# ziatdinovmax/pyroVED

Measured on AMD Instinct MI355X. Metric: images/sec (SVI step), higher is better.
Workload: dtype bf16; 1 GPU; C2 iVAE 28x28 invariances=['r','t'] latent_dim=2 bernoulli, batch 256 per GPU (global 256), bf16 MFMA operands for the hidden-layer contractions (fp32 accumulate; fp32 elsewhere); the guide (fc encoder, sample, split) runs in the decoder launch's prologue in fp32, SVI step = ELBO+grads+Adam; parallelism=dp1

## Files before the change

pyroved_amd/csrc/pv_sdec_fused_w8.hip:

```cpp
#include "pv_sdec_fused.h"
#include "pv_fb_layout.h"
#include "pv_sdec_prims.h"
#include "pv_kernels.h"
#include <stdlib.h>

#define W8_WAVES 8
#define W8_ROWS (W8_WAVES * FD_UNIT)
#define W8_THREADS (64 * W8_WAVES)
#define W8_ARR (W8_ROWS * LDS2)
#define W8_ARR_BYTES (2 * W8_ARR)
#define WO_W1 0
#define WO_W2 IMG_BYTES
#define WO_SA (2 * IMG_BYTES)
#define WO_SB (WO_SA + W8_ARR_BYTES)
#define WO_VEC (WO_SB + W8_ARR_BYTES)
#define WO_ATAB (WO_VEC + 3 * FD_H * 4)
#define WO_TTAB (WO_ATAB + 8 * 64 * 8)
#define WO_INFO (WO_TTAB + 4 * 64 * 16)
#define WO_RED (WO_INFO + 3 * W8_ROWS * 4)
#define WO_CHZ (WO_RED + 256)
#define WO_CTP (WO_CHZ + W8_WAVES * FD_H * 4)
#define WO_CGR (WO_CTP + W8_WAVES * 256)
#define W8_LDS_BYTES (WO_CGR + W8_WAVES * 256)
#define WO_TX (WO_SB + 2 * 32 * LDS2)
// ... 2 lines not shown
static_assert(WO_TLOG + W8_WAVES * 16 * 4 <= WO_SB + W8_ARR_BYTES, "tail exchange buffers fit behind the staged rows");
static_assert(W8_LDS_BYTES <= 160 * 1024, "LDS budget");
static_assert(2 * IMG_BYTES % (W8_WAVES * 1024) == 0, "image load: whole 1 KB LDS-DMA pieces per wave");

#ifndef W8_FENCE_MASK
#define W8_FENCE_MASK 0
#endif
#define W8_FENCE() __builtin_amdgcn_sched_barrier(W8_FENCE_MASK)

__device__ __forceinline__ float w8_tanhc(float cx) {
  const float e = __builtin_amdgcn_exp2f(cx);
  return 1.0f - 2.0f * __builtin_amdgcn_rcpf(e + 1.0f);
}
#ifndef W8_HSWAP
#define W8_HSWAP 0
#endif
#ifndef W8_QSWAP
#define W8_QSWAP 1
#endif
bool pv_sdec_fused_w8_qswap() { return W8_QSWAP != 0; }
__device__ __forceinline__ bf16x8 w8_catq(const bf16x4& a, const bf16x4& b, int q) {
  return W8_QSWAP ? sd_catq(a, b, q >= 2) : sd_cat(a, b);
}
__device__ __forceinline__ float w8_sum_q(float v) {
  return pv_sum_rows(v);
}

#ifndef W8_ABL
#define W8_ABL 0
#endif
#ifndef W8_TAIL
#define W8_TAIL 1
#endif
#define W8_ABL_LOADS(bit, g) (!(W8_ABL & (bit)) || (((g) & 1) == 0))
#define W8_ABL_BUF(bit, g) ((W8_ABL & (bit)) ? (((g) >> 1) & 1) : ((g) & 1))


struct W8Addr : SdAddr { int fs, hs; };
__device__ __forceinline__ W8Addr w8_addr(int r, int q) {
  W8Addr a;
  a.fs = W8_HSWAP ? ((r >> 2) & 1) : 0;
  a.hs = W8_HSWAP ? (q & 1) : (W8_QSWAP ? ((r >> 1) & 1) : 0);
  static_cast<SdAddr&>(a) = sd_addr(r, q);
  return a;
}

__device__ __forceinline__ void w8_layer_fwd(const __bf16* __restrict__ Wh, const float* __restrict__ bs,
                                             const bf16x4 (&ih)[8], f32x4 (&out)[8], const W8Addr& ad, int q) {
#pragma unroll
  for (int ob = 0; ob < 8; ++ob) out[ob] = *reinterpret_cast<const f32x4*>(bs + 16 * ob + 4 * q);
  const __bf16* ah = Wh + ad.fb;
#if W8_HSWAP
  const __bf16* ah0 = ah + 4 * ad.fs;
  const __bf16* ah1 = ah + 4 - 4 * ad.fs;
  asm volatile("" : "+v"(ah0), "+v"(ah1));
#endif
  const int (&xm)[4] = ad.fx;
  bf16x8 wh[2][2];
  auto load = [&](int g, bf16x8 (&h)[2]) {
    const int m = g >> 2, op = (g & 3) * 2;
#pragma unroll
    for (int o = 0; o < 2; ++o) {
#if W8_HSWAP
      typedef const volatile bf16x4* vp4;
      const bf16x4 lo4 = *reinterpret_cast<vp4>(ah0 + 16 * (op + o) * LDB + xm[m]);
      const bf16x4 hi4 = *reinterpret_cast<vp4>(ah1 + 16 * (op + o) * LDB + xm[m]);
// ... 183 lines not shown
}
__device__ __forceinline__ f32x4 w8_tanh4(f32x4 v) {
#pragma unroll
  for (int i = 0; i < 4; ++i) v[i] = w8_tanhc(v[i]);
  return v;
}
__device__ __forceinline__ bf16x4 w8_cvt4(const f32x4& v) {
  bf16x4 h;
#pragma unroll
  for (int i = 0; i < 4; ++i) h[i] = (__bf16)v[i];
  return h;
}
__device__ __forceinline__ f32x4 w8_mul_dtanh4(const f32x4& d, const bf16x4& hb) {
  const f32x4 t = sd_f32_of(hb);
  return d * (t * t - 1.0f);
}

#define WF_H1 WO_SA
#define WF_H2 (WF_H1 + 512)
#define WF_HD (WF_H2 + 512)
#define WF_P (WF_HD + 512)
#define WF_P_WAVE (64 * 17 * 4)
static_assert(WF_P + W8_WAVES * WF_P_WAVE <= WO_VEC, "guide scratch fits in the staging arrays");
#include "pv_gemv16.h"

#define W8_COOP_SPINS 4096
__device__ unsigned w8_coop_late_total;
extern "C" int pv_debug_coop_late_count(unsigned* out) {
  return (int)hipMemcpyFromSymbol(out, HIP_SYMBOL(w8_coop_late_total), sizeof(unsigned));
}
template <bool GRADS, int LIK, int FOLDK>
__global__ __launch_bounds__(W8_THREADS) void pv_sdec_w8_kernel(PvFused f, PvEncFold e) {
  constexpr bool FOLD = FOLDK != 0, CHAIN = FOLDK >= 2, COOP = FOLDK == 3;
  extern __shared__ __attribute__((aligned(16))) char smb[];
  const int tid = threadIdx.x, lane0 = tid & 63, lane = lane0, r = lane & 15, q = lane >> 4;
  const int wave = __builtin_amdgcn_readfirstlane(tid >> 6);
  const int g = blockIdx.x, G = gridDim.x;
  const unsigned lds0 = __builtin_amdgcn_readfirstlane((unsigned)(size_t)smb);
  const __bf16* W1h = reinterpret_cast<const __bf16*>(smb + WO_W1);
  const __bf16* W2h = reinterpret_cast<const __bf16*>(smb + WO_W2);
  __bf16* sA = reinterpret_cast<__bf16*>(smb + WO_SA);
  __bf16* sB = reinterpret_cast<__bf16*>(smb + WO_SB);
  float* vec = reinterpret_cast<float*>(smb + WO_VEC);
  float* info = reinterpret_cast<float*>(smb + WO_INFO);
  float* red = reinterpret_cast<float*>(smb + WO_RED);
  const char* gimg = reinterpret_cast<const char*>(f.wimg);
  W8_STAMP_K(0);
  f32x4 xr[4], xpk;
  f32x4 xc[4][4];
  unsigned coop_tag = 0;
  if (COOP) {
    coop_tag = e.coop_flags[G] + 1u;
    const int K4 = (int)(e.ldx >> 2);
#pragma unroll
    for (int i = 0; i < 4; ++i) {
      const float* xg = e.x + (int64_t)(8 * (4 * wave + i) + (g & 7)) * e.ldx;
#pragma unroll
      for (int c = 0; c < 4; ++c) {
        const int k4 = lane + 64 * c;
        xc[i][c] = *reinterpret_cast<const f32x4*>(xg + 4 * (k4 < K4 ? k4 : 0));
      }
    }
  }
  if (FOLD && !COOP) {
    const int K4 = (int)(e.ldx >> 2);
    const float* xg = e.x + (int64_t)g * e.ldx;
#pragma unroll
    for (int c = 0; c < 4; ++c) {
      const int k4 = lane + 64 * c;
      xr[c] = *reinterpret_cast<const f32x4*>(xg + 4 * (k4 < K4 ? k4 : 0));
    }
    const int kp = 64 * (((K4 + 63) >> 6) - 1) + (lane & 3);
    xpk = *reinterpret_cast<const f32x4*>(xg + 4 * (kp < K4 ? kp : 0));
  }
  float pt_v[3] = {0.0f, 0.0f, 0.0f}, pt_a = 0.0f, pt_t[8] = {0.0f, 0.0f, 0.0f, 0.0f, 0.0f, 0.0f, 0.0f, 0.0f};
  if (FOLD) {
    if (tid < FD_H) { pt_v[0] = f.wo[tid]; pt_v[1] = f.b1[tid]; pt_v[2] = f.b2[tid]; }
    {
      const int jb = tid >> 6, m = lane & 15, kq = lane >> 4, j = 16 * jb + m;
      if (kq == 0) pt_a = f.Wc[j * f.cd];
      else if (kq == 1) pt_a = f.cd == 2 ? f.Wc[j * 2 + 1] : 0.0f;
      else if (kq == 2) pt_a = f.bc[j];
    }
    if (tid < 256) {
      const int mm = tid >> 6, m = lane & 15, kq = lane >> 4;
#pragma unroll
      for (int e_ = 0; e_ < 8; ++e_) {
        const int j = 32 * mm + 4 * kq + (e_ < 4 ? e_ : 16 + e_ - 4);
        if (m < 2) pt_t[e_] = f.Wc[j * f.cd];
        else if (m < 4 && f.cd == 2) pt_t[e_] = f.Wc[j * 2 + 1];
      }
    }
  }

  f32x4 w1v[8], w2v[8];
  if (!FOLD) {
    constexpr int PIECES = IMG_BYTES / (W8_WAVES * 1024);
#pragma unroll
    for (int c = 0; c < PIECES; ++c) {
      const int off = (wave * PIECES + c) * 1024;
      sd_glds16(gimg + off + lane * 16, lds0 + WO_W1 + off);
      sd_glds16(gimg + 2 * IMG_BYTES + off + lane * 16, lds0 + WO_W2 + off);
    }
  } else {
    if (GRADS) {
      const int64_t b0 = (int64_t)g * e.img_per_wg;
      f32x4* zp = reinterpret_cast<f32x4*>(f.part_hz + b0 * f.kmax * FD_H);
      const int n4 = e.img_per_wg * f.kmax * (FD_H / 4);
      for (int i = tid; i < n4; i += W8_THREADS) zp[i] = f32x4{0.0f, 0.0f, 0.0f, 0.0f};
      if (f.part_rs) {
        f32x4* zr = reinterpret_cast<f32x4*>(f.part_rs + b0 * f.kmax * PV_RS_W);
        for (int i = tid; i < e.img_per_wg * f.kmax * (PV_RS_W / 4); i += W8_THREADS) zr[i] = f32x4{0.0f, 0.0f, 0.0f, 0.0f};
      }
    }
  }
  if (FOLD) {
    float* h1s = reinterpret_cast<float*>(smb + WF_H1);
    float* h2s = reinterpret_cast<float*>(smb + WF_H2);
    float* hds = reinterpret_cast<float*>(smb + WF_HD);
    float* zs = hds + 64;
    float* P = reinterpret_cast<float*>(smb + WF_P + wave * WF_P_WAVE);
    const int N = (int)e.ldx, zd = e.z_dim;
    const int r_ = lane & 15, q_ = lane >> 4;
    {
      const int64_t b = g;
      const int jw = 16 * wave + r_;
      const float pb1 = (e.enc1.b_off >= 0 && jw < e.enc1.out_dim) ? e.params[e.enc1.b_off + jw] : 0.0f;
      const float pbh = (e.head.b_off >= 0 && jw < e.head.out_dim) ? e.params[e.head.b_off + jw] : 0.0f;
      const float pep = (wave == 0 && lane < zd) ? e.eps[b * zd + lane] : 0.0f;
      f32x4 wl1[8], wlh[8];
      float pwz[4] = {0.0f, 0.0f, 0.0f, 0.0f};
      if (tid < FD_H) {
#pragma unroll
        for (int i = 0; i < 4; ++i) pwz[i] = i < e.lat_in ? e.Wz[(int64_t)tid * e.lat_in + i] : 0.0f;
      }
      auto layer0_alone = [&](const f32x4 (&xr_)[4], const f32x4& xpk_, bool load_next) {
        const int jr = 16 * ((wave + g) & (W8_WAVES - 1));
        const float v = w8_gemv16(e.params + e.enc0.w_off, N, e.enc0.out_dim, jr, xr_, xpk_, P, lane,
// ... 155 lines not shown
      }
      pv_lds_barrier();
      if (tid < FD_H) {
        int coord = 0;
        if (e.coord_dim == 1) coord = e.has_t ? 1 : 0;
        else if (e.coord_dim == 2) coord = e.has_r + 2 * e.has_t + e.has_s;
        const float* wz = e.Wz + (int64_t)tid * e.lat_in;
        float v = 0.0f;
        for (int i = 0; i < e.lat_in; ++i) v += zs[coord + i] * (i < 4 ? pwz[i] : wz[i]);
        e.hz[b * FD_H + tid] = v * SD_C;
      }
      W8_STAMP_K(7);
    }
  }
  if (tid < FD_H) {
    vec[tid] = FOLD ? pt_v[0] : f.wo[tid];
    vec[FD_H + tid] = SD_C * (FOLD ? pt_v[1] : f.b1[tid]);
    vec[2 * FD_H + tid] = SD_C * (FOLD ? pt_v[2] : f.b2[tid]);
  }
  {
    const int jb = tid >> 6, m = lane & 15, kq = lane >> 4, j = 16 * jb + m;
    float v = 0.0f;
    if (FOLD) v = SD_C * pt_a;
    else if (kq == 0) v = SD_C * f.Wc[j * f.cd];
    else if (kq == 1) v = f.cd == 2 ? SD_C * f.Wc[j * 2 + 1] : 0.0f;
    else if (kq == 2) v = SD_C * f.bc[j];
    __bf16 hi, lo;
    fb_split(v, hi, lo);
    bf16x4 a = sd_zero4();
    if (kq < 2) { a[0] = hi; a[1] = hi; a[2] = lo; }
    else if (kq == 2) { a[0] = hi; a[1] = lo; }
    reinterpret_cast<bf16x4*>(smb + WO_ATAB)[tid] = a;
  }
  if (tid < 256) {
    const int mm = tid >> 6, m = lane & 15, kq = lane >> 4;
    bf16x8 a;
#pragma unroll
    for (int e = 0; e < 8; ++e) {
      const int j = 32 * mm + 4 * kq + (e < 4 ? e : 16 + e - 4);
      float w = 0.0f;
      if (FOLD) w = pt_t[e];
      else if (m < 2) w = f.Wc[j * f.cd];
      else if (m < 4 && f.cd == 2) w = f.Wc[j * 2 + 1];
      __bf16 hi, lo;
      fb_split(w, hi, lo);
      a[e] = m >= 4 ? (__bf16)0.0f : ((m & 1) ? lo : hi);
    }
    reinterpret_cast<bf16x8*>(smb + WO_TTAB)[tid] = a;
  }
  if (FOLD) {
    typedef unsigned short us4 __attribute__((ext_vector_type(4)));
    __bf16* i1 = reinterpret_cast<__bf16*>(smb + WO_W1);
    __bf16* i2 = reinterpret_cast<__bf16*>(smb + WO_W2);
#pragma unroll
    for (int u = 0; u < 8; ++u) {
      const int idx = tid + W8_THREADS * u, row = idx >> 5, c4 = idx & 31;
      us4 h1, h2;
#pragma unroll
      for (int i = 0; i < 4; ++i) {
        h1[i] = __builtin_bit_cast(unsigned short, (__bf16)(w1v[u][i] * SD_C));
        h2[i] = __builtin_bit_cast(unsigned short, (__bf16)(w2v[u][i] * SD_C));
      }
      const int el = fb_wel(row, fb_pcol(4 * c4)) ^ (W8_HSWAP ? 4 * ((row >> 2) & 1) : 0) ^ (W8_QSWAP ? 4 * ((c4 >> 1) & 1) : 0);
      *reinterpret_cast<us4*>(i1 + el) = h1;
      *reinterpret_cast<us4*>(i2 + el) = h2;
    }
  }
  sd_wait_vm0();
  __syncthreads();
  W8_STAMP_K(1);
  const float bo = f.bo[0];
  typedef __attribute__((address_space(1))) float gfloat;
  unsigned long long u_llrow, u_loc, u_rowtp, u_part_hz;
  int64_t a_M;
  asm volatile("s_mov_b64 %0, %5\n\ts_mov_b64 %1, %6\n\ts_mov_b64 %2, %7\n\ts_mov_b64 %3, %8\n\ts_mov_b64 %4, %9"
               : "=&s"(u_llrow), "=&s"(u_loc), "=&s"(u_rowtp), "=&s"(u_part_hz), "=&s"(a_M)
               : "s"((unsigned long long)f.llrow), "s"((unsigned long long)f.loc), "s"((unsigned long long)f.rowtp),
                 "s"((unsigned long long)f.part_hz), "s"(f.M));
  gfloat* a_llrow = (gfloat*)u_llrow; gfloat* a_loc = (gfloat*)u_loc; gfloat* a_rowtp = (gfloat*)u_rowtp;
  gfloat* a_part_hz = (gfloat*)u_part_hz;

  f32x4 accW1[2][4], accW2[2][4], accS[8], accB1 = {0, 0, 0, 0}, accB2 = {0, 0, 0, 0};
#pragma unroll
  for (int kb = 0; kb < 8; ++kb) {
    accW1[kb >> 2][kb & 3] = f32x4{0, 0, 0, 0}; accW2[kb >> 2][kb & 3] = f32x4{0, 0, 0, 0}; accS[kb] = f32x4{0, 0, 0, 0};
  }
  float dbo = 0.0f;
  int cur_b = -1;
  const int upb = f.N / FD_UNIT;
  float* rec = f.part + (int64_t)g * FD_REC;

  auto flush_hz = [&](int b) {
    const int64_t ub = (int64_t)b * upb;
    const int gfirst = (int)(((ub + 1) * G + f.units - 1) / f.units) - 1;
    gfloat* dst = a_part_hz + ((int64_t)b * f.kmax + (g - gfirst) * W8_WAVES + wave) * FD_H + 4 * q;
    if (r == 0) {
#pragma unroll
      for (int jb = 0; jb < 8; ++jb) *(__attribute__((address_space(1))) f32x4*)(dst + 16 * jb) = accS[jb] * SD_RC2;
    }
#pragma unroll
    for (int jb = 0; jb < 8; ++jb)
#pragma unroll
      for (int i = 0; i < 4; ++i) accS[jb][i] = r == 0 ? 0.0f : accS[jb][i];
  };

  const int u_lo = (int)((int64_t)g * f.units / G), u_hi = (int)((int64_t)(g + 1) * f.units / G);
  const int xun = (int)f.x_units;
  struct Pos { int unit, b, loc, xu; };
  auto pos_of = [&](int unit_) {
    Pos p_;
    p_.unit = unit_; p_.b = unit_ / upb; p_.loc = unit_ - p_.b * upb; p_.xu = xun > 0 ? unit_ % xun : unit_;
    return p_;
  };
  auto advance = [&](Pos& p_, int by) {
    p_.unit += by; p_.loc += by; p_.xu += by;
    while (p_.loc >= upb) { p_.loc -= upb; ++p_.b; }
    if (xun > 0) { while (p_.xu >= xun) p_.xu -= xun; }
  };
  const bool has_tail = W8_TAIL && ((u_hi - u_lo) & (W8_WAVES - 1)) == 1;
  const int u_end = has_tail ? u_hi - 1 : u_hi;
  const Pos pos_lo = pos_of(has_tail ? u_end : u_lo);
  Pos pos_cur = pos_of(u_lo + wave < u_end ? u_lo + wave : (has_tail ? u_end : u_lo));
  Pos pos_nx = pos_cur;
  float sw_next = 1.0f;
  auto x_of = [&](const Pos& p_) -> float {
    if (f.sw) sw_next = f.sw[p_.b];
    return f.x[(int64_t)p_.xu * FD_UNIT + r];
  };
  float xv_next = x_of(pos_cur);
  float* chz = reinterpret_cast<float*>(smb + WO_CHZ) + wave * FD_H;
  float* ctp = reinterpret_cast<float*>(smb + WO_CTP) + wave * 64;
  float* cgr = reinterpret_cast<float*>(smb + WO_CGR) + wave * 64;
  auto fetch_unit_inputs = [&](const Pos& p_) {
    const int n0 = p_.loc * FD_UNIT;
    sd_glds4(f.hz + (int64_t)p_.b * FD_H + lane, lds0 + WO_CHZ + wave * (FD_H * 4));
    sd_glds4(f.hz + (int64_t)p_.b * FD_H + 64 + lane, lds0 + WO_CHZ + wave * (FD_H * 4) + 256);
    sd_glds4(f.tp + (int64_t)p_.b * 8 + (lane & 7), lds0 + WO_CTP + wave * 256);
    sd_glds4(f.grid + (int64_t)n0 * f.cd + (lane & (16 * f.cd - 1)), lds0 + WO_CGR + wave * 256);
  };
  fetch_unit_inputs(pos_cur);
  const W8Addr wad = w8_addr(r, q);
  int tile_no = -1;
  for (int ut = u_lo; ut < u_end; ut += W8_WAVES) {
    ++tile_no;
    (void)tile_no;
    asm volatile("; W8_TILE_BEGIN");
    W8_STAMP(0);
    const int nact = (u_end - ut) < W8_WAVES ? (u_end - ut) : W8_WAVES;
    if (ut + W8_WAVES + wave < u_end) advance(pos_nx, W8_WAVES);
    else pos_nx = pos_lo;
    int opq = 0;
    asm volatile("" : "+v"(opq));
    const int lane = lane0 | opq, r = lane & 15, q = lane >> 4;
    const float* wos = vec;
    const float* b1s = vec + FD_H;
    const float* b2s = vec + 2 * FD_H;
    const bool act = wave < nact;
    const int unit = act ? pos_cur.unit : ut;
    const int bu = pos_cur.b;
    const int64_t row = (int64_t)unit * FD_UNIT + r;
    float x0, x1, u0c, u1c, sc;
    sd_wait_vm0();
    {
      const float* t = ctp;
      const float* gr = cgr;
      if (f.cd == 2) {
        const float gx = gr[2 * r], gy = gr[2 * r + 1];
        u0c = gx * t[0] - gy * t[1];
        u1c = gx * t[1] + gy * t[0];
        sc = t[2];
        x0 = u0c * sc + t[3];
        x1 = u1c * sc + t[4];
      } else {
// ... 12 lines not shown
    {
      bf16x4 bx = sd_zero4();
      {
        const float v = q == 0 ? x0 : x1;
        __bf16 vh, vl;
        fb_split(v, vh, vl);
        const __bf16 one = (__bf16)1.0f;
        if (q < 2) { bx[0] = vh; bx[1] = vl; bx[2] = vh; }
        else if (q == 2) { bx[0] = one; bx[1] = one; }
      }
      const bf16x4* atab = reinterpret_cast<const bf16x4*>(smb + WO_ATAB) + lane;
      const float* hzb = chz;
      bf16x4 aop[8];
#pragma unroll
      for (int jb = 0; jb < 8; ++jb) {
        tC[jb] = *reinterpret_cast<const f32x4*>(hzb + 16 * jb + 4 * q);
        aop[jb] = atab[64 * jb];
      }
      if (GRADS && q == 0) { inf_x0[r] = x0; inf_x1[r] = x1; }
      W8_FENCE();
      if (f.hz_scale == 0.0f) {
#pragma unroll
        for (int jb = 0; jb < 8; ++jb) tC[jb] = tC[jb] * SD_C;
      }
      W8_FENCE();
#pragma unroll
      for (int jb = 0; jb < 8; ++jb) tC[jb] = sd_mfma16(aop[jb], bx, tC[jb]);
      W8_FENCE();
      sd_tanh8<W8_FENCE_MASK>(tC);
      w8_cvt8(tC, h0b);
    }
    asm volatile("; W8_P1_coord_done");
    W8_STAMP(1);
    fetch_unit_inputs(pos_nx);
    {
      w8_layer_fwd(W1h, b1s, h0b, tC, wad, q);
      sd_tanh8<W8_FENCE_MASK>(tC);
      w8_cvt8(tC, h1b);
      asm volatile("; W8_P2_l1_done");
    W8_STAMP(2);
      w8_layer_fwd(W2h, b2s, h1b, tC, wad, q);
      sd_tanh8<W8_FENCE_MASK>(tC);
      f32x4 part4 = {0.0f, 0.0f, 0.0f, 0.0f};
#pragma unroll
      for (int jb = 0; jb < 8; ++jb) {
        const f32x4 wv = *reinterpret_cast<const f32x4*>(wos + 16 * jb + 4 * q);
        part4 = part4 + tC[jb] * wv;
        if (GRADS) {
#pragma unroll
          for (int i = 0; i < 4; ++i) pA[jb][i] = (__bf16)tC[jb][i];
          const f32x4 t2 = tC[jb] * tC[jb];
          tC[jb] = wv - wv * t2;
        }
      }
      const float a = w8_sum_q((part4[0] + part4[1]) + (part4[2] + part4[3])) + bo;
      float ll, locv;
      sd_pixel_lik<LIK>(a, xv, f.sig, f.sigmoid_out, ll, dlda, locv);
      dlda *= act ? swv : 0.0f;
      if (q == 0) {
        if (act) {
          if (a_llrow) a_llrow[row] = ll;
          if (a_loc) a_loc[row] = locv;
        }
        if (GRADS) { dbo += dlda; inf_dl[r] = dlda; }
      }
      xv_next = x_of(pos_nx);
    }
    pos_cur = pos_nx;
    asm volatile("; W8_P3_fwd_done");
    W8_STAMP(3);
    if (!GRADS) continue;
    const int ksteps = (nact + 1) >> 1;
    {
      sd_wait_lgkm0();
      const f32x4 d4 = *reinterpret_cast<const f32x4*>(inf_dl + 4 * q);
      bf16x4 bw = sd_zero4();
#pragma unroll
      for (int i = 0; i < 4; ++i) {
        __bf16 hi, lo;
        fb_split(d4[i], hi, lo);
        bw[i] = r == 3 ? hi : (r == 4 ? lo : (__bf16)0.0f);
      }
      w8_colsum_mfma(sA, pA, bw, accS, wave, r, q);
#pragma unroll
      for (int jb = 0; jb < 8; ++jb) tC[jb] = tC[jb] * dlda;
      w8_cvt8(tC, pA);
    }
    asm volatile("; W8_P4_dwo_done");
    W8_STAMP(4);
    sd_stage_store(sA, pA, 16 * wave + r, q);
    sd_stage_store(sB, h1b, 16 * wave + r, q);
    __syncthreads();
    asm volatile("; W8_P5_bar1");
    W8_STAMP(5);
    w8_wgrad_consume(sA, sB, accW2, accB2, wave, r, q, ksteps);
    asm volatile("; W8_P6_cons2");
    W8_STAMP(6);
    bf16x4 p0[8];
    {
      w8_layer_dgrad(W2h, pA, tC, wad);
      w8_mul_dtanh(tC, h1b);
      w8_cvt8(tC, pA);
      asm volatile("; W8_P7_dgrad2");
    W8_STAMP(7);
      w8_layer_dgrad(W1h, pA, tC, wad);
      w8_mul_dtanh(tC, h0b);
      w8_cvt8(tC, p0);
    }
    asm volatile("; W8_P8_dgrad1");
    W8_STAMP(8);
    __syncthreads();
    W8_STAMP(9);
    {
      f32x4 dd = {0.0f, 0.0f, 0.0f, 0.0f};
      const bf16x8* ttab = reinterpret_cast<const bf16x8*>(smb + WO_TTAB) + lane;
#pragma unroll
      for (int mm = 0; mm < 4; ++mm) dd = MFMA32(ttab[64 * mm], sd_cat(p0[2 * mm], p0[2 * mm + 1]), dd);
      if (q == 0 && act) {
        const float d0 = (dd[0] + dd[1]) * SD_RC2, d1 = (dd[2] + dd[3]) * SD_RC2;
        a_rowtp[row] = sc * (d1 * u0c - d0 * u1c);
        a_rowtp[a_M + row] = d0 * u0c + d1 * u1c;
        a_rowtp[2 * a_M + row] = d0;
        a_rowtp[3 * a_M + row] = d1;
      }
      if (act && bu != cur_b) {
        if (cur_b >= 0) flush_hz(cur_b);
        cur_b = bu;
      }
      const f32x4 a0 = *reinterpret_cast<const f32x4*>(inf_x0 + 4 * q);
      const f32x4 a1 = *reinterpret_cast<const f32x4*>(inf_x1 + 4 * q);
      bf16x4 bc_ = sd_zero4();
      const bool use1 = r == 2 || r == 6, lo_col = r >= 5;
#pragma unroll
      for (int i = 0; i < 4; ++i) {
        __bf16 hi, lo;
        fb_split(use1 ? a1[i] : a0[i], hi, lo);
        __bf16 v = lo_col ? lo : hi;
        if (r == 0) v = (__bf16)1.0f;
        if (r == 3 || r == 4 || r > 6) v = (__bf16)0.0f;
        bc_[i] = v;
      }
      w8_colsum_mfma(sA, p0, bc_, accS, wave, r, q);
      sd_wait_lgkm0();
    }
    asm volatile("; W8_P12_rowlocal");
    W8_STAMP(12);
    sd_stage_store(sA, pA, 16 * wave + r, q);
    sd_stage_store(sB, h0b, 16 * wave + r, q);
    __syncthreads();
    asm volatile("; W8_P10_bar3");
    W8_STAMP(10);
    w8_wgrad_consume(sA, sB, accW1, accB1, wave, r, q, ksteps);
    asm volatile("; W8_P11_cons1");
    W8_STAMP(11);
    __syncthreads();
    asm volatile("; W8_P13_bar4");
    W8_STAMP(13);
    W8_STAMP(14);
    asm volatile("; W8_TILE_END");
  }
// ... 65 lines not shown
      }
      float* tlog = reinterpret_cast<float*>(smb + WO_TLOG);
      if (q == 0) tlog[16 * wave + r] = part;
      __syncthreads();
      float a = bo;
      {
        float sacc = 0.0f;
#pragma unroll
        for (int w = 0; w < W8_WAVES; ++w) sacc += tlog[16 * w + r];
        a += sacc;
      }
      float ll, locv;
      if (LIK == PV_LIK_BERNOULLI) {
        const float pr = sd_rcp(1.0f + sd_exp(-a));
        const float pc = fminf(fmaxf(pr, BERN_EPS), 1.0f - BERN_EPS);
        const float lpc = sd_log(pc), l1pc = sd_log(1.0f - pc);
        const float lg = lpc - l1pc;
        ll = -(fmaxf(lg, 0.0f) - lg * xv - fmaxf(lpc, l1pc));
        const float mask = (pr >= BERN_EPS && pr <= 1.0f - BERN_EPS) ? 1.0f : 0.0f;
        dlda = (pc - xv) * mask;
        locv = pr;
      } else if (LIK == PV_LIK_CBERNOULLI) {
        pv_cbern(a, xv, ll, dlda, locv);
      } else {
        const float pr = f.sigmoid_out ? sd_rcp(1.0f + sd_exp(-a)) : a;
        const float d = xv - pr;
        ll = -(d * d) / (2.0f * f.sig * f.sig) - sd_log(f.sig) - LOG_SQRT_2PI;
        dlda = -d / (f.sig * f.sig) * (f.sigmoid_out ? pr * (1.0f - pr) : 1.0f);
        locv = pr;
      }
      dlda *= swv;
      if (q == 0) {
        if (wave == 0) {
          if (a_llrow) a_llrow[row] = ll;
          if (a_loc) a_loc[row] = locv;
          if (GRADS) dbo += dlda;
        }
        if (GRADS) inf_dl[r] = dlda;
      }
    }
    if (GRADS) {
      bf16x4 pA[8];
      w8_xchg_put(smb, 3, w8_cvt4(gq * dlda), wave, lane);
      __syncthreads();
      w8_xchg_get(smb, 3, pA, lane);
      if (wave == 0) {
        sd_stage_store(sA, pA, r, q);
        sd_stage_store(sB, h1b, r, q);
      } else if (wave == 1) {
        bf16x4 z8[8];
#pragma unroll
        for (int jb = 0; jb < 8; ++jb) z8[jb] = sd_zero4();
        sd_stage_store(sA, z8, 16 + r, q);
        sd_stage_store(sB, h1b, 16 + r, q);
      } else if (wave == 3) {
        bf16x4 h2b[8];
        w8_xchg_get(smb, 2, h2b, lane);
        sd_wait_lgkm0();
        const f32x4 d4 = *reinterpret_cast<const f32x4*>(inf_dl + 4 * q);
        bf16x4 bw = sd_zero4();
#pragma unroll
        for (int i = 0; i < 4; ++i) {
          __bf16 hi, lo;
          fb_split(d4[i], hi, lo);
          bw[i] = r == 3 ? hi : (r == 4 ? lo : (__bf16)0.0f);
        }
        w8_colsum_mfma(sA, h2b, bw, accS, wave, r, q);
      }
      const f32x4 d1 = w8_mul_dtanh4(w8_tail_dgrad(W2h, pA, wad, wave, r), own1);
      w8_xchg_put(smb, 4, w8_cvt4(d1), wave, lane);
      __syncthreads();
      w8_xchg_get(smb, 4, pA, lane);
      w8_wgrad_consume(sA, sB, accW2, accB2, wave, r, q, 1);
      const f32x4 d0 = w8_mul_dtanh4(w8_tail_dgrad(W1h, pA, wad, wave, r), own0);
      w8_xchg_put(smb, 5, w8_cvt4(d0), wave, lane);
      __syncthreads();
      if (wave == 0) {
        sd_stage_store(sA, pA, r, q);
        sd_stage_store(sB, h0b, r, q);
      } else if (wave == 1) {
        bf16x4 z8[8];
#pragma unroll
        for (int jb = 0; jb < 8; ++jb) z8[jb] = sd_zero4();
        sd_stage_store(sA, z8, 16 + r, q);
        sd_stage_store(sB, h0b, 16 + r, q);
      } else if (wave == 2) {
        bf16x4 p0[8];
        w8_xchg_get(smb, 5, p0, lane);
        f32x4 dd = {0.0f, 0.0f, 0.0f, 0.0f};
        const bf16x8* ttab = reinterpret_cast<const bf16x8*>(smb + WO_TTAB) + lane;
#pragma unroll
        for (int mm = 0; mm < 4; ++mm) dd = MFMA32(ttab[64 * mm], sd_cat(p0[2 * mm], p0[2 * mm + 1]), dd);
        if (q == 0) {
          const float d0_ = (dd[0] + dd[1]) * SD_RC2, d1_ = (dd[2] + dd[3]) * SD_RC2;
          a_rowtp[row] = sc * (d1_ * u0c - d0_ * u1c);
          a_rowtp[a_M + row] = d0_ * u0c + d1_ * u1c;
          a_rowtp[2 * a_M + row] = d0_;
          a_rowtp[3 * a_M + row] = d1_;
        }
      } else if (wave == 3) {
        bf16x4 p0[8];
        w8_xchg_get(smb, 5, p0, lane);
        if (bu != cur_b) {
          if (cur_b >= 0) flush_hz(cur_b);
          cur_b = bu;
        }
        const f32x4 a0 = *reinterpret_cast<const f32x4*>(inf_x0 + 4 * q);
        const f32x4 a1 = *reinterpret_cast<const f32x4*>(inf_x1 + 4 * q);
        bf16x4 bc_ = sd_zero4();
        const bool use1 = r == 2 || r == 6, lo_col = r >= 5;
#pragma unroll
        for (int i = 0; i < 4; ++i) {
          __bf16 hi, lo;
          fb_split(use1 ? a1[i] : a0[i], hi, lo);
          __bf16 v = lo_col ? lo : hi;
          if (r == 0) v = (__bf16)1.0f;
          if (r == 3 || r == 4 || r > 6) v = (__bf16)0.0f;
          bc_[i] = v;
        }
        w8_colsum_mfma(sA, p0, bc_, accS, wave, r, q);
      }
      __syncthreads();
      w8_wgrad_consume(sA, sB, accW1, accB1, wave, r, q, 1);
    }
    asm volatile("; W8_TAIL_END");
  }
  if (!GRADS) return;
  W8_STAMP_K(2);

  const PvEncFoldArg ep_ = pv_kernarg_fold();
  const bool own_dhz = FOLD && f.dhz_out != nullptr;
  if (cur_b >= 0 && !own_dhz) flush_hz(cur_b);
  W8_STAMP_E(0);
  __syncthreads();
  W8_STAMP_E(1);
  float rsv[2][5] = {{0.0f, 0.0f, 0.0f, 0.0f, 0.0f}, {0.0f, 0.0f, 0.0f, 0.0f, 0.0f}};
  const bool fold_rs = FOLD && f.part_rs && f.N <= 2 * W8_THREADS && f.N % 2 == 0;
  if (fold_rs) {
    const int64_t r0 = (int64_t)g * f.N;
    if (2 * tid < f.N) {
      auto ld2 = [](const float* p_, float& a, float& b) {
        const unsigned long long v = __hip_atomic_load(reinterpret_cast<const unsigned long long*>(p_), __ATOMIC_RELAXED, __HIP_MEMORY_SCOPE_AGENT);
        a = __uint_as_float((unsigned)v); b = __uint_as_float((unsigned)(v >> 32));
      };
      ld2(f.llrow + r0 + 2 * tid, rsv[0][0], rsv[1][0]);
#pragma unroll
      for (int c = 0; c < 4; ++c) ld2(f.rowtp + (int64_t)c * f.M + r0 + 2 * tid, rsv[0][1 + c], rsv[1][1 + c]);
    }
  }
  W8_STAMP_E(10);
  float wzv[4] = {0.0f, 0.0f, 0.0f, 0.0f};
  if (FOLD && f.dhz_out && f.dzc_out && tid < FD_H) {
#pragma unroll
    for (int i = 0; i < 4; ++i) wzv[i] = i < ep_->lat_in ? ep_->Wz[(int64_t)tid * ep_->lat_in + i] : 0.0f;
  }
  const bool own_chain = CHAIN && ep_->chain && f.part_rs && f.dhz_out && f.dzc_out;
  float ch_whd[16], ch_a1 = 0.0f, ch_a0 = 0.0f, ch_z = 0.0f, ch_sig = 1.0f, ch_ep = 0.0f, ch_sp = 0.0f;
  f32x4 ch_w1[8];
  if (own_chain) {
    auto ldc = [](const float* p_) { return __hip_atomic_load(p_, __ATOMIC_RELAXED, __HIP_MEMORY_SCOPE_AGENT); };
    const int ho = ep_->head.out_dim;
    if (tid < FD_H) {
      const float* Wh = ep_->params + ep_->head.w_off + tid;
#pragma unroll
      for (int o = 0; o < 16; ++o) ch_whd[o] = Wh[(o < ho ? o : ho - 1) * FD_H];
      ch_a1 = ldc(ep_->eact1 + (int64_t)g * FD_H + tid);
      ch_a0 = ldc(ep_->eact0 + (int64_t)g * FD_H + tid);
    }
    const float* W1c = ep_->params + ep_->enc1.w_off + 4 * (tid & 31) + (8 * (tid >> 5)) * FD_H;
#pragma unroll
    for (int jj = 0; jj < 8; ++jj) ch_w1[jj] = *reinterpret_cast<const f32x4*>(W1c + jj * FD_H);
    if (lane < ep_->z_dim && wave < 2) {
      ch_z = ldc(ep_->z + (int64_t)g * ep_->z_dim + lane);
      ch_sig = ldc(ep_->z_scale + (int64_t)g * ep_->z_dim + lane);
      ch_ep = ep_->eps[(int64_t)g * ep_->z_dim + lane];
      ch_sp = ldc(ep_->head_out + (int64_t)g * ep_->ldh + ep_->z_dim + lane);
    }
  }
  W8_STAMP_E(11);
  {
    const int jp = wave >> 1, kh = wave & 1;
    auto pack2 = [](float a, float b) {
      typedef __bf16 bf2_ __attribute__((ext_vector_type(2)));
      bf2_ h; h[0] = (__bf16)a; h[1] = (__bf16)b;
      return __builtin_bit_cast(unsigned, h);
    };
    if (f.ablate & 1024) {
#pragma unroll
      for (int s_ = 0; s_ < 2; ++s_)
#pragma unroll
        for (int o = 0; o < 4; ++o)
#pragma unroll
          for (int i = 0; i < 4; ++i) {
// ... 8 lines not shown
      for (int s_ = 0; s_ < 2; ++s_)
#pragma unroll
        for (int o = 0; o < 4; ++o) {
          u32x4_ v;
          v[0] = pack2(accW1[s_][o][0] * -SD_RC, accW1[s_][o][1] * -SD_RC);
          v[1] = pack2(accW1[s_][o][2] * -SD_RC, accW1[s_][o][3] * -SD_RC);
          v[2] = pack2(accW2[s_][o][0], accW2[s_][o][1]);
          v[3] = pack2(accW2[s_][o][2], accW2[s_][o][3]);
          rec4[((wave * 2 + s_) * 4 + o) * 64 + lane] = v;
        }
    }
    if (r == 0) {
      const int j0 = 32 * jp + 16 * kh;
#pragma unroll
      for (int i = 0; i < 4; ++i) {
        rec[2 * FD_H * FD_H + j0 + 4 * q + i] = accB1[i] * -SD_RC;
        rec[2 * FD_H * FD_H + FD_H + j0 + 4 * q + i] = accB2[i];
      }
    }
  }
  W8_STAMP_E(12);
  {
    float* scr = reinterpret_cast<float*>(smb + WO_SA);
#pragma unroll
    for (int jb = 0; jb < 8; ++jb)
      *reinterpret_cast<f32x4*>(scr + ((wave * 16 + r) * FD_H) + 16 * jb + 4 * q) = accS[jb];
  }
  const float tb = pv_wave_sum(dbo);
  if (lane == 0) red[wave] = tb;
  W8_STAMP_E(2);
  pv_lds_barrier();
  W8_STAMP_E(3);
  float dhz_j = 0.0f;
  if (tid < FD_H) {
    const float* scr = reinterpret_cast<const float*>(smb + WO_SA);
    float vo = 0.0f, v0 = 0.0f, v1 = 0.0f, vh = 0.0f;
#pragma unroll
    for (int w = 0; w < W8_WAVES; ++w) {
      const float* s_ = scr + (w * 16) * FD_H + tid;
      vh += s_[0];
      v0 += s_[1 * FD_H] + s_[5 * FD_H];
      v1 += s_[2 * FD_H] + s_[6 * FD_H];
      vo += s_[3 * FD_H] + s_[4 * FD_H];
    }
    dhz_j = vh * SD_RC2;
    if (own_dhz) f.dhz_out[(int64_t)g * FD_H + tid] = dhz_j;
    rec[2 * FD_H * FD_H + 2 * FD_H + tid] = v0 * SD_RC2;
    rec[2 * FD_H * FD_H + 3 * FD_H + tid] = v1 * SD_RC2;
    rec[2 * FD_H * FD_H + 4 * FD_H + tid] = vo;
  }
  const bool own_dzc = own_dhz && f.dzc_out != nullptr;
  if (FOLD && (f.part_rs || own_dzc)) {
    if (f.part_rs) {
      const int64_t r0 = (int64_t)g * f.N;
      float a5[5] = {0.0f, 0.0f, 0.0f, 0.0f, 0.0f};
      if (fold_rs) {
#pragma unroll
        for (int c = 0; c < 5; ++c) a5[c] = rsv[0][c] + rsv[1][c];
      } else {
        for (int n = tid; n < f.N; n += W8_THREADS) {
          a5[0] += __hip_atomic_load(f.llrow + r0 + n, __ATOMIC_RELAXED, __HIP_MEMORY_SCOPE_AGENT);
#pragma unroll
          for (int c = 0; c < 4; ++c) a5[1 + c] += __hip_atomic_load(f.rowtp + (int64_t)c * f.M + r0 + n, __ATOMIC_RELAXED, __HIP_MEMORY_SCOPE_AGENT);
        }
      }
#pragma unroll
      for (int c = 0; c < 5; ++c) a5[c] = pv_wave_sum(a5[c]);
      if (lane == 0) {
#pragma unroll
        for (int c = 0; c < 5; ++c) red[8 + 8 * c + wave] = a5[c];
      }
    }
    if (own_dzc && wave < 2) {
      for (int i = 0; i < ep_->lat_in; ++i) {
        const float pz = pv_wave_sum(dhz_j * (i < 4 ? wzv[i] : ep_->Wz[(int64_t)tid * ep_->lat_in + i]));
        if (lane == 0) info[16 * wave + i] = pz;
      }
    }
    W8_STAMP_E(4);
    pv_lds_barrier();
    W8_STAMP_E(5);
    float* cs = reinterpret_cast<float*>(smb + WO_SA);
    if (f.part_rs && tid < 5) {
      float v = 0.0f;
      for (int w = 0; w < W8_WAVES; ++w) v += red[8 + 8 * tid + w];
      f.part_rs[((int64_t)g * f.kmax) * PV_RS_W + tid] = v;
    }
    if (own_dzc && tid < ep_->lat_in) f.dzc_out[(int64_t)g * ep_->lat_in + tid] = info[tid] + info[16 + tid];
    if (own_chain) {
      if (wave < 2) {
        float* csw = cs + 64 * wave;
        if (lane < 5) {
          float v = 0.0f;
#pragma unroll
          for (int w = 0; w < W8_WAVES; ++w) v += red[8 + 8 * lane + w];
          csw[lane] = v;
          if (tid == 0) ep_->llb[g] = v;
        }
        if (lane >= 8 && lane < 8 + ep_->lat_in) csw[lane] = info[lane - 8] + info[16 + lane - 8];
        asm volatile("s_waitcnt lgkmcnt(0)" ::: "memory");
        PvHeadBwd hb{};
        hb.coord_dim = ep_->coord_dim; hb.has_r = ep_->has_r; hb.has_t = ep_->has_t; hb.has_s = ep_->has_s;
        hb.tp0 = ep_->tp0; hb.tp1 = ep_->tp1; hb.sc_prior = ep_->sc_prior;
        if (lane < 16) {
          float g_ = 0.0f, ds_ = 0.0f;
          if (lane < ep_->z_dim) {
            const float dz = pv_head_dz(hb, lane, [&](int c) { return csw[1 + c]; }, [&](int k) { return csw[8 + k]; });
            pv_head_bwd_math(dz, ch_z, ch_sig, ch_ep, ch_sp, ep_->beta, 0, g_, ds_);
            if (wave == 0) {
              ep_->dhead[(int64_t)g * ep_->ldh + lane] = g_;
              ep_->dhead[(int64_t)g * ep_->ldh + ep_->z_dim + lane] = ds_;
            }
            csw[16 + lane] = g_;
            csw[16 + ep_->z_dim + lane] = ds_;
          } else if (lane + ep_->z_dim < 16) {
            csw[16 + ep_->z_dim + lane] = 0.0f;
          }
        }
        asm volatile("s_waitcnt lgkmcnt(0)" ::: "memory");
        float v = 0.0f;
#pragma unroll
        for (int o = 0; o < 16; ++o) v += csw[16 + o] * ch_whd[o];
        v *= pv_act_grad2(ch_a1, 0.0f, ep_->enc1.act);
        ep_->edp1[(int64_t)g * FD_H + tid] = v;
        cs[128 + tid] = v;
      }
      pv_lds_barrier();
      W8_STAMP_E(6);
// ... 21 lines not shown
    for (int w = 0; w < W8_WAVES; ++w) v += red[w];
    rec[2 * FD_H * FD_H + 5 * FD_H] = v;
  }
  W8_STAMP_K(3);
}

bool pv_sdec_fused_w8_fold_ok(const PvFused& f, int grid) {
  if (f.N % FD_UNIT != 0 || f.N > 1024 || f.N % 4 != 0 || grid < 1 || f.B % grid != 0 || f.x_units != 0) return false;
  const int ipw = f.B / grid;
  return ipw == 1 && f.units == (int64_t)f.B * (f.N / FD_UNIT);
}

int pv_sdec_fused_w8_launch(const PvFused& f_in, int grid, bool grads, hipStream_t s, const PvEncFold* fold) {
  PvFused f = f_in;
  static const int ablate = pv_exp_int("PV_FD_ABLATE", 0) & 1024;
  f.ablate = ablate;
  const size_t lds = W8_LDS_BYTES;
  const void* fn = nullptr;
  PvEncFold e{};
  if (fold) {
    if (!pv_sdec_fused_w8_fold_ok(f, grid)) return PV_EINVAL;
    e = *fold;
    e.img_per_wg = f.B / grid;
    if (e.coop && !(grid == 256 && e.enc0.out_dim == FD_H && e.coop_flags && e.chain)) e.coop = 0;
#ifndef PV_EXPERIMENTS
    e.coop = 0;
#endif
  }
#ifdef PV_EXPERIMENTS
#define W8_COOP_BUILD 3
#else
#define W8_COOP_BUILD 2
#endif
#define W8_PICK(G, L) fn = !fold ? reinterpret_cast<const void*>(&pv_sdec_w8_kernel<G, L, 0>)                     \
                               : (G && e.chain && e.coop) ? reinterpret_cast<const void*>(&pv_sdec_w8_kernel<G, L, G ? W8_COOP_BUILD : 1>) \
                               : (G && e.chain) ? reinterpret_cast<const void*>(&pv_sdec_w8_kernel<G, L, G ? 2 : 1>) \
                                                : reinterpret_cast<const void*>(&pv_sdec_w8_kernel<G, L, 1>)
  if (grads) {
    if (f.lik == PV_LIK_BERNOULLI) W8_PICK(true, PV_LIK_BERNOULLI);
    else if (f.lik == PV_LIK_GAUSSIAN) W8_PICK(true, PV_LIK_GAUSSIAN);
    else W8_PICK(true, PV_LIK_CBERNOULLI);
  } else {
    if (f.lik == PV_LIK_BERNOULLI) W8_PICK(false, PV_LIK_BERNOULLI);
    else if (f.lik == PV_LIK_GAUSSIAN) W8_PICK(false, PV_LIK_GAUSSIAN);
    else W8_PICK(false, PV_LIK_CBERNOULLI);
  }
#undef W8_PICK
  PV_TRY(pv_set_dynamic_lds(fn, (int)lds));
  void* args[] = {&f, &e};
  hipError_t e2 = hipLaunchKernel(fn, dim3(grid), dim3(W8_THREADS), args, lds, s);
  if (e2 != hipSuccess) return (int)e2;
  PV_LAUNCH_CHECK();
  return 0;
}
```

Baseline: 2.681 million images/s.

## Derive per-image row sums from reduced gradients instead of per-row buffers in chained grad path

In the chained gradient kernel, per-row log-likelihood and per-row transform partials (llrow, rowtp) are no longer written to global memory and re-read. The kernel now accumulates the log-likelihood in a register and computes the rotation and translation sums algebraically from the already-reduced dWc and dhz vectors. This also skips zeroing and flushing part_hz, the per-unit hz/tp refetches, and the TTAB MFMA. It removes global traffic and per-row work, but the algebraic identity ties correctness to the single-image-per-workgroup layout, and the launcher now rejects chained calls that lack part_rs, dhz_out or dzc_out.

```diff
diff --git a/pyroved_amd/csrc/pv_sdec_fused_w8.hip b/pyroved_amd/csrc/pv_sdec_fused_w8.hip
--- a/pyroved_amd/csrc/pv_sdec_fused_w8.hip
+++ b/pyroved_amd/csrc/pv_sdec_fused_w8.hip
@@ -58,6 +58,9 @@
 #ifndef W8_TAIL
 #define W8_TAIL 1
 #endif
+#ifndef W8_OWN_SUMS
+#define W8_OWN_SUMS 1
+#endif
 #define W8_ABL_LOADS(bit, g) (!(W8_ABL & (bit)) || (((g) & 1) == 0))
 #define W8_ABL_BUF(bit, g) ((W8_ABL & (bit)) ? (((g) >> 1) & 1) : ((g) & 1))
 
@@ -307,6 +310,7 @@
 template <bool GRADS, int LIK, int FOLDK>
 __global__ __launch_bounds__(W8_THREADS) void pv_sdec_w8_kernel(PvFused f, PvEncFold e) {
   constexpr bool FOLD = FOLDK != 0, CHAIN = FOLDK >= 2, COOP = FOLDK == 3;
+  constexpr bool OWN = W8_OWN_SUMS && CHAIN && GRADS;
   extern __shared__ __attribute__((aligned(16))) char smb[];
   const int tid = threadIdx.x, lane0 = tid & 63, lane = lane0, r = lane & 15, q = lane >> 4;
   const int wave = __builtin_amdgcn_readfirstlane(tid >> 6);
@@ -357,7 +361,7 @@
       else if (kq == 1) pt_a = f.cd == 2 ? f.Wc[j * 2 + 1] : 0.0f;
       else if (kq == 2) pt_a = f.bc[j];
     }
-    if (tid < 256) {
+    if (!OWN && tid < 256) {
       const int mm = tid >> 6, m = lane & 15, kq = lane >> 4;
 #pragma unroll
       for (int e_ = 0; e_ < 8; ++e_) {
@@ -378,7 +382,7 @@
       sd_glds16(gimg + 2 * IMG_BYTES + off + lane * 16, lds0 + WO_W2 + off);
     }
   } else {
-    if (GRADS) {
+    if (GRADS && !OWN) {
       const int64_t b0 = (int64_t)g * e.img_per_wg;
       f32x4* zp = reinterpret_cast<f32x4*>(f.part_hz + b0 * f.kmax * FD_H);
       const int n4 = e.img_per_wg * f.kmax * (FD_H / 4);
@@ -600,7 +604,7 @@
     else if (kq == 2) { a[0] = hi; a[1] = lo; }
     reinterpret_cast<bf16x4*>(smb + WO_ATAB)[tid] = a;
   }
-  if (tid < 256) {
+  if (!OWN && tid < 256) {
     const int mm = tid >> 6, m = lane & 15, kq = lane >> 4;
     bf16x8 a;
 #pragma unroll
@@ -639,12 +643,16 @@
   W8_STAMP_K(1);
   const float bo = f.bo[0];
   typedef __attribute__((address_space(1))) float gfloat;
-  unsigned long long u_llrow, u_loc, u_rowtp, u_part_hz;
-  int64_t a_M;
-  asm volatile("s_mov_b64 %0, %5\n\ts_mov_b64 %1, %6\n\ts_mov_b64 %2, %7\n\ts_mov_b64 %3, %8\n\ts_mov_b64 %4, %9"
-               : "=&s"(u_llrow), "=&s"(u_loc), "=&s"(u_rowtp), "=&s"(u_part_hz), "=&s"(a_M)
-               : "s"((unsigned long long)f.llrow), "s"((unsigned long long)f.loc), "s"((unsigned long long)f.rowtp),
-                 "s"((unsigned long long)f.part_hz), "s"(f.M));
+  unsigned long long u_llrow = 0, u_loc, u_rowtp = 0, u_part_hz = 0;
+  int64_t a_M = 0;
+  if constexpr (OWN) {
+    asm volatile("s_mov_b64 %0, %1" : "=&s"(u_loc) : "s"((unsigned long long)f.loc));
+  } else {
+    asm volatile("s_mov_b64 %0, %5\n\ts_mov_b64 %1, %6\n\ts_mov_b64 %2, %7\n\ts_mov_b64 %3, %8\n\ts_mov_b64 %4, %9"
+                 : "=&s"(u_llrow), "=&s"(u_loc), "=&s"(u_rowtp), "=&s"(u_part_hz), "=&s"(a_M)
+                 : "s"((unsigned long long)f.llrow), "s"((unsigned long long)f.loc), "s"((unsigned long long)f.rowtp),
+                   "s"((unsigned long long)f.part_hz), "s"(f.M));
+  }
   gfloat* a_llrow = (gfloat*)u_llrow; gfloat* a_loc = (gfloat*)u_loc; gfloat* a_rowtp = (gfloat*)u_rowtp;
   gfloat* a_part_hz = (gfloat*)u_part_hz;
 
@@ -654,6 +662,7 @@
     accW1[kb >> 2][kb & 3] = f32x4{0, 0, 0, 0}; accW2[kb >> 2][kb & 3] = f32x4{0, 0, 0, 0}; accS[kb] = f32x4{0, 0, 0, 0};
   }
   float dbo = 0.0f;
+  float llacc = 0.0f;
   int cur_b = -1;
   const int upb = f.N / FD_UNIT;
   float* rec = f.part + (int64_t)g * FD_REC;
@@ -699,14 +708,16 @@
   float* chz = reinterpret_cast<float*>(smb + WO_CHZ) + wave * FD_H;
   float* ctp = reinterpret_cast<float*>(smb + WO_CTP) + wave * 64;
   float* cgr = reinterpret_cast<float*>(smb + WO_CGR) + wave * 64;
-  auto fetch_unit_inputs = [&](const Pos& p_) {
+  auto fetch_unit_inputs = [&](const Pos& p_, bool first) {
     const int n0 = p_.loc * FD_UNIT;
-    sd_glds4(f.hz + (int64_t)p_.b * FD_H + lane, lds0 + WO_CHZ + wave * (FD_H * 4));
-    sd_glds4(f.hz + (int64_t)p_.b * FD_H + 64 + lane, lds0 + WO_CHZ + wave * (FD_H * 4) + 256);
-    sd_glds4(f.tp + (int64_t)p_.b * 8 + (lane & 7), lds0 + WO_CTP + wave * 256);
+    if (!OWN || first) {
+      sd_glds4(f.hz + (int64_t)p_.b * FD_H + lane, lds0 + WO_CHZ + wave * (FD_H * 4));
+      sd_glds4(f.hz + (int64_t)p_.b * FD_H + 64 + lane, lds0 + WO_CHZ + wave * (FD_H * 4) + 256);
+      sd_glds4(f.tp + (int64_t)p_.b * 8 + (lane & 7), lds0 + WO_CTP + wave * 256);
+    }
     sd_glds4(f.grid + (int64_t)n0 * f.cd + (lane & (16 * f.cd - 1)), lds0 + WO_CGR + wave * 256);
   };
-  fetch_unit_inputs(pos_cur);
+  fetch_unit_inputs(pos_cur, true);
   const W8Addr wad = w8_addr(r, q);
   int tile_no = -1;
   for (int ut = u_lo; ut < u_end; ut += W8_WAVES) {
@@ -785,7 +796,7 @@
     }
     asm volatile("; W8_P1_coord_done");
     W8_STAMP(1);
-    fetch_unit_inputs(pos_nx);
+    fetch_unit_inputs(pos_nx, false);
     {
       w8_layer_fwd(W1h, b1s, h0b, tC, wad, q);
       sd_tanh8<W8_FENCE_MASK>(tC);
@@ -812,7 +823,8 @@
       dlda *= act ? swv : 0.0f;
       if (q == 0) {
         if (act) {
-          if (a_llrow) a_llrow[row] = ll;
+          if constexpr (OWN) llacc += ll;
+          else if (a_llrow) a_llrow[row] = ll;
           if (a_loc) a_loc[row] = locv;
         }
         if (GRADS) { dbo += dlda; inf_dl[r] = dlda; }
@@ -865,20 +877,22 @@
     __syncthreads();
     W8_STAMP(9);
     {
-      f32x4 dd = {0.0f, 0.0f, 0.0f, 0.0f};
-      const bf16x8* ttab = reinterpret_cast<const bf16x8*>(smb + WO_TTAB) + lane;
-#pragma unroll
-      for (int mm = 0; mm < 4; ++mm) dd = MFMA32(ttab[64 * mm], sd_cat(p0[2 * mm], p0[2 * mm + 1]), dd);
-      if (q == 0 && act) {
-        const float d0 = (dd[0] + dd[1]) * SD_RC2, d1 = (dd[2] + dd[3]) * SD_RC2;
-        a_rowtp[row] = sc * (d1 * u0c - d0 * u1c);
-        a_rowtp[a_M + row] = d0 * u0c + d1 * u1c;
-        a_rowtp[2 * a_M + row] = d0;
-        a_rowtp[3 * a_M + row] = d1;
-      }
-      if (act && bu != cur_b) {
-        if (cur_b >= 0) flush_hz(cur_b);
-        cur_b = bu;
+      if constexpr (!OWN) {
+        f32x4 dd = {0.0f, 0.0f, 0.0f, 0.0f};
+        const bf16x8* ttab = reinterpret_cast<const bf16x8*>(smb + WO_TTAB) + lane;
+#pragma unroll
+        for (int mm = 0; mm < 4; ++mm) dd = MFMA32(ttab[64 * mm], sd_cat(p0[2 * mm], p0[2 * mm + 1]), dd);
+        if (q == 0 && act) {
+          const float d0 = (dd[0] + dd[1]) * SD_RC2, d1 = (dd[2] + dd[3]) * SD_RC2;
+          a_rowtp[row] = sc * (d1 * u0c - d0 * u1c);
+          a_rowtp[a_M + row] = d0 * u0c + d1 * u1c;
+          a_rowtp[2 * a_M + row] = d0;
+          a_rowtp[3 * a_M + row] = d1;
+        }
+        if (act && bu != cur_b) {
+          if (cur_b >= 0) flush_hz(cur_b);
+          cur_b = bu;
+        }
       }
       const f32x4 a0 = *reinterpret_cast<const f32x4*>(inf_x0 + 4 * q);
       const f32x4 a1 = *reinterpret_cast<const f32x4*>(inf_x1 + 4 * q);
@@ -1010,7 +1024,8 @@
       dlda *= swv;
       if (q == 0) {
         if (wave == 0) {
-          if (a_llrow) a_llrow[row] = ll;
+          if constexpr (OWN) llacc += ll;
+          else if (a_llrow) a_llrow[row] = ll;
           if (a_loc) a_loc[row] = locv;
           if (GRADS) dbo += dlda;
         }
@@ -1062,7 +1077,7 @@
         for (int jb = 0; jb < 8; ++jb) z8[jb] = sd_zero4();
         sd_stage_store(sA, z8, 16 + r, q);
         sd_stage_store(sB, h0b, 16 + r, q);
-      } else if (wave == 2) {
+      } else if (!OWN && wave == 2) {
         bf16x4 p0[8];
         w8_xchg_get(smb, 5, p0, lane);
         f32x4 dd = {0.0f, 0.0f, 0.0f, 0.0f};
@@ -1079,7 +1094,7 @@
       } else if (wave == 3) {
         bf16x4 p0[8];
         w8_xchg_get(smb, 5, p0, lane);
-        if (bu != cur_b) {
+        if (!OWN && bu != cur_b) {
           if (cur_b >= 0) flush_hz(cur_b);
           cur_b = bu;
         }
@@ -1108,12 +1123,13 @@
 
   const PvEncFoldArg ep_ = pv_kernarg_fold();
   const bool own_dhz = FOLD && f.dhz_out != nullptr;
-  if (cur_b >= 0 && !own_dhz) flush_hz(cur_b);
+  if (!OWN && cur_b >= 0 && !own_dhz) flush_hz(cur_b);
   W8_STAMP_E(0);
-  __syncthreads();
+  if constexpr (OWN) pv_lds_barrier();
+  else __syncthreads();
   W8_STAMP_E(1);
   float rsv[2][5] = {{0.0f, 0.0f, 0.0f, 0.0f, 0.0f}, {0.0f, 0.0f, 0.0f, 0.0f, 0.0f}};
-  const bool fold_rs = FOLD && f.part_rs && f.N <= 2 * W8_THREADS && f.N % 2 == 0;
+  const bool fold_rs = !OWN && FOLD && f.part_rs && f.N <= 2 * W8_THREADS && f.N % 2 == 0;
   if (fold_rs) {
     const int64_t r0 = (int64_t)g * f.N;
     if (2 * tid < f.N) {
@@ -1135,8 +1151,13 @@
   const bool own_chain = CHAIN && ep_->chain && f.part_rs && f.dhz_out && f.dzc_out;
   float ch_whd[16], ch_a1 = 0.0f, ch_a0 = 0.0f, ch_z = 0.0f, ch_sig = 1.0f, ch_ep = 0.0f, ch_sp = 0.0f;
   f32x4 ch_w1[8];
+  float wc0 = 0.0f, wc1 = 0.0f;
+  if (OWN && tid < FD_H) {
+    wc0 = f.Wc[tid * f.cd];
+    if (f.cd == 2) wc1 = f.Wc[tid * 2 + 1];
+  }
   if (own_chain) {
-    auto ldc = [](const float* p_) { return __hip_atomic_load(p_, __ATOMIC_RELAXED, __HIP_MEMORY_SCOPE_AGENT); };
+    auto ldc =[](const float* p_) { return __hip_atomic_load(p_, __ATOMIC_RELAXED, __HIP_MEMORY_SCOPE_AGENT); };
     const int ho = ep_->head.out_dim;
     if (tid < FD_H) {
       const float* Wh = ep_->params + ep_->head.w_off + tid;
@@ -1211,6 +1232,7 @@
   pv_lds_barrier();
   W8_STAMP_E(3);
   float dhz_j = 0.0f;
+  float dwc0_j = 0.0f, dwc1_j = 0.0f;
   if (tid < FD_H) {
     const float* scr = reinterpret_cast<const float*>(smb + WO_SA);
     float vo = 0.0f, v0 = 0.0f, v1 = 0.0f, vh = 0.0f;
@@ -1223,14 +1245,30 @@
       vo += s_[3 * FD_H] + s_[4 * FD_H];
     }
     dhz_j = vh * SD_RC2;
+    dwc0_j = v0 * SD_RC2;
+    dwc1_j = v1 * SD_RC2;
     if (own_dhz) f.dhz_out[(int64_t)g * FD_H + tid] = dhz_j;
-    rec[2 * FD_H * FD_H + 2 * FD_H + tid] = v0 * SD_RC2;
-    rec[2 * FD_H * FD_H + 3 * FD_H + tid] = v1 * SD_RC2;
+    rec[2 * FD_H * FD_H + 2 * FD_H + tid] = dwc0_j;
+    rec[2 * FD_H * FD_H + 3 * FD_H + tid] = dwc1_j;
     rec[2 * FD_H * FD_H + 4 * FD_H + tid] = vo;
   }
   const bool own_dzc = own_dhz && f.dzc_out != nullptr;
   if (FOLD && (f.part_rs || own_dzc)) {
-    if (f.part_rs) {
+    if (OWN && f.part_rs) {
+      const float lw = pv_wave_sum(llacc);
+      if (lane == 0) red[8 + wave] = lw;
+      if (wave < 2) {
+        const float tx = ctp[3], ty = f.cd == 2 ? ctp[4] : 0.0f;
+        const float a_ = dwc0_j - tx * dhz_j, b_ = dwc1_j - ty * dhz_j;
+        const float s4[4] = {wc1 * a_ - wc0 * b_, wc0 * a_ + wc1 * b_, wc0 * dhz_j, wc1 * dhz_j};
+#pragma unroll
+        for (int c = 0; c < 4; ++c) {
+          const float s_ = pv_wave_sum(s4[c]);
+          if (lane == 0) red[16 + 8 * wave + c] = s_;
+        }
+      }
+    }
+    if (!OWN && f.part_rs) {
       const int64_t r0 = (int64_t)g * f.N;
       float a5[5] = {0.0f, 0.0f, 0.0f, 0.0f, 0.0f};
       if (fold_rs) {
@@ -1260,19 +1298,29 @@
     pv_lds_barrier();
     W8_STAMP_E(5);
     float* cs = reinterpret_cast<float*>(smb + WO_SA);
-    if (f.part_rs && tid < 5) {
+    auto row_sum = [&](int c) {
       float v = 0.0f;
-      for (int w = 0; w < W8_WAVES; ++w) v += red[8 + 8 * tid + w];
-      f.part_rs[((int64_t)g * f.kmax) * PV_RS_W + tid] = v;
-    }
+      if constexpr (OWN) {
+        if (c == 0) {
+#pragma unroll
+          for (int w = 0; w < W8_WAVES; ++w) v += red[8 + w];
+        } else {
+          v = red[16 + c - 1] + red[24 + c - 1];
+          if (c == 2 && f.cd == 2) v /= ctp[2];
+        }
+      } else {
+#pragma unroll
+        for (int w = 0; w < W8_WAVES; ++w) v += red[8 + 8 * c + w];
+      }
+      return v;
+    };
+    if (f.part_rs && tid < 5) f.part_rs[((int64_t)g * f.kmax) * PV_RS_W + tid] = row_sum(tid);
     if (own_dzc && tid < ep_->lat_in) f.dzc_out[(int64_t)g * ep_->lat_in + tid] = info[tid] + info[16 + tid];
     if (own_chain) {
       if (wave < 2) {
         float* csw = cs + 64 * wave;
         if (lane < 5) {
-          float v = 0.0f;
-#pragma unroll
-          for (int w = 0; w < W8_WAVES; ++w) v += red[8 + 8 * lane + w];
+          const float v = row_sum(lane);
           csw[lane] = v;
           if (tid == 0) ep_->llb[g] = v;
         }
@@ -1360,9 +1408,11 @@
 #else
 #define W8_COOP_BUILD 2
 #endif
+  const bool chain = fold && e.chain;
+  if (chain && grads && !(f.part_rs && f.dhz_out && f.dzc_out)) return PV_EINVAL;
 #define W8_PICK(G, L) fn = !fold ? reinterpret_cast<const void*>(&pv_sdec_w8_kernel<G, L, 0>)                     \
-                               : (G && e.chain && e.coop) ? reinterpret_cast<const void*>(&pv_sdec_w8_kernel<G, L, G ? W8_COOP_BUILD : 1>) \
-                               : (G && e.chain) ? reinterpret_cast<const void*>(&pv_sdec_w8_kernel<G, L, G ? 2 : 1>) \
+                               : (G && chain && e.coop) ? reinterpret_cast<const void*>(&pv_sdec_w8_kernel<G, L, G ? W8_COOP_BUILD : 1>) \
+                               : (G && chain) ? reinterpret_cast<const void*>(&pv_sdec_w8_kernel<G, L, G ? 2 : 1>) \
                                                 : reinterpret_cast<const void*>(&pv_sdec_w8_kernel<G, L, 1>)
   if (grads) {
     if (f.lik == PV_LIK_BERNOULLI) W8_PICK(true, PV_LIK_BERNOULLI);
```

After: 2.783 million images/s, median of 6. 1.04x the previous value.
